# marcin119a/vae-los-angeles

Hardware: AMD Instinct MI355X
Metric: training samples/sec, MultiModalVAE batch 65536 (higher is better)
Workload: dtype bf16

## Files before the change

### include/mmvae_hip.h

```cpp
#ifndef MMVAE_HIP_H
#define MMVAE_HIP_H
#include <stdint.h>

#ifdef __cplusplus
extern "C" {
#endif

#define MMVAE_OK 0
#define MMVAE_ERR_ARG (-1)
#define MMVAE_ERR_DTYPE (-2)

enum { MMVAE_F32 = 0, MMVAE_BF16 = 1 };
enum { MMVAE_PREC_F32 = 0, MMVAE_PREC_BF16 = 1 };
enum { MMVAE_PRO_NONE = 0, MMVAE_PRO_BN_RELU_DROP = 1, MMVAE_PRO_BN_BWD_APPLY = 2 };
enum { MMVAE_EPI_STORE = 0, MMVAE_EPI_RELU_MASK = 1, MMVAE_EPI_BN_BWD = 2, MMVAE_EPI_LOSS_MSE = 3, MMVAE_EPI_LOSS_BCE_LOGIT = 4 };
enum { MMVAE_ACT_NONE = 0, MMVAE_ACT_RELU = 1, MMVAE_ACT_SIGMOID = 2 };

#define MMVAE_TILE 128

int mmvae_abi_version(void);
int mmvae_set_tuning(int32_t key, int32_t value);

typedef struct {
    const float* src; void* dst;
// ... 101 lines not shown
    const void* w; int64_t ldw; const float* bias;
} mmvae_latent_enc;
typedef struct {
    int32_t prec, B, L, n_mod;
    mmvae_latent_enc enc_a, enc_b;
    const float* table; const int64_t* site; int32_t S;
    const float* eps;
    float* mu; float* logvar;
    void* z; int64_t ldz;
    const void* w_stem; int64_t ldw_stem; const float* bias_stem; int32_t N_stem;
    void* h0; int64_t ldh0;
} mmvae_latent_fwd_args;
int mmvae_latent_fwd(const mmvae_latent_fwd_args* args, void* stream);

typedef struct {
    int32_t B, A, D, S, L;
    const float* recon_a; const void* a; int64_t ld_ra, ld_a;
    const float* recon_b; const void* b; int64_t ld_rb, ld_b;
    const float* logits; int64_t ld_logits; const int64_t* site; const float* class_weights;
    const float* mu; const float* logvar;
    float beta, gamma;
    double* sums;
    void* g_a; int32_t g_a_dtype; int64_t ld_ga;
    void* g_b; int32_t g_b_dtype; int64_t ld_gb; int32_t grad_b_wrt_logit;
    float* g_c; int64_t ld_gc;
    float* g_mu; float* g_lv;
    const float* beta_gamma_dev;
    int32_t a_dtype, b_dtype;
} mmvae_loss_args;
int mmvae_vae_loss(const mmvae_loss_args* args, void* stream);
// ... 33 lines not shown
```

### vae-los-angeles_amd/csrc/common.h

```cpp
#pragma once
#include <hip/hip_runtime.h>
#include <stdint.h>
#include "mmvae_hip.h"

namespace mm {

typedef __bf16 bf16;
typedef __attribute__((ext_vector_type(8))) __bf16 bf16x8;
typedef __attribute__((ext_vector_type(4))) __bf16 bf16x4;
typedef __attribute__((ext_vector_type(4))) float f32x4;
typedef __attribute__((ext_vector_type(2))) float f32x2;
typedef __attribute__((ext_vector_type(4))) short s16x4;

constexpr int WAVE = 64;
constexpr int TILE = 128;
constexpr int NTHREADS = 256;
constexpr int ROW_BYTES = 128;

template <typename CT> struct Mma;

template <> struct Mma<bf16> {
    static constexpr int EPC = 8;
    static constexpr int KSTEP = 32;
    typedef bf16x8 frag;
// ... 124 lines not shown
#define STAMP_ENTRY()
#endif


struct Tuning {
    int nt_wide_min_m = 256 * 128;
    int nt2_on = 1;
    long split_bytes = 1L << 32;
    long block_bytes = 1L << 31;
    int tn_wide_on = 1;
    int bnbwd_stream = 1;
    int relu_stream = 1;
    int ntp_on = 1;
    int ntp_min_m = 16384;
    int latent_on = 1;
};
inline Tuning g_tuning;

constexpr int NOT_TAKEN = 1 << 30;

template <auto Kernel, typename... Args>
inline int launch_lds(dim3 grid, dim3 block, int lds, hipStream_t st, const Args&... args) {
    static bool attr_done = false;
    if (!attr_done) {
        hipError_t e = hipFuncSetAttribute((const void*)Kernel, hipFuncAttributeMaxDynamicSharedMemorySize, lds);
        if (e != hipSuccess) return (int)e;
        attr_done = true;
    }
    hipLaunchKernelGGL(Kernel, grid, block, lds, st, args...);
    return (int)hipGetLastError();
// ... 49 lines not shown
```

### vae-los-angeles_amd/csrc/elementwise.hip

```cpp
#include <vector>
#include "common.h"
#include "mmvae_hip.h"
#include "fuse_math.h"

namespace mm {

__global__ __launch_bounds__(256) void prep_weights_kernel(const mmvae_prep_item* __restrict__ items) {
    const mmvae_prep_item it = items[blockIdx.y];
    __shared__ float tile[32][33];
    const int tx = threadIdx.x & 31, ty = threadIdx.x >> 5;
    const int tiles_c = (it.dst_cols + 31) / 32, tiles_r = (it.dst_rows + 31) / 32;
    auto put = [&](int r, int c, float v) {
        if (it.dst_dtype == MMVAE_BF16) ((bf16*)it.dst)[(long)r * it.dst_ld + c] = (bf16)v;
        else ((float*)it.dst)[(long)r * it.dst_ld + c] = v;
    };
    for (int t = blockIdx.x; t < tiles_r * tiles_c; t += gridDim.x) {
        const int tr = t / tiles_c, tc = t - tr * tiles_c;
        if (it.transpose) {
#pragma unroll
            for (int k = 0; k < 4; ++k) {
                const int sr = tc * 32 + ty + 8 * k, sc = tr * 32 + tx;
                tile[ty + 8 * k][tx] = (sr < it.src_rows && sc < it.src_cols) ? it.src[(long)sr * it.src_ld + sc] : 0.f;
            }
            __syncthreads();
// ... 226 lines not shown
            const long i = min(i0 + (long)u * blockDim.x, iend - 1);
            const int b = (int)(i / a.L), l = (int)(i - (long)b * a.L);
            bb[u] = b; ll[u] = l;
            dz[u] = a.dz[(long)b * a.lddz + l];
            if (a.dz2) dz[u] += a.dz2[(long)b * a.lddz + l];
            if (a.dz3) dz[u] += a.dz3[(long)b * a.lddz + l];
            gm[u] = a.g_mu ? a.g_mu[i] : 0.f; gl[u] = a.g_lv ? a.g_lv[i] : 0.f;
            ep[u] = a.eps[i]; lv[u] = a.logvar[i];
            sidx[u] = a.d_table ? a.site[b] : 0;
            if (sidx[u] < 0 || sidx[u] >= a.S) sidx[u] = -1;
        }
#pragma unroll
        for (int u = 0; u < U; ++u) {
            if (i0 + (long)u * blockDim.x >= iend) break;
            const int b = bb[u], l = ll[u];
            float dmu = gm[u] + dz[u];
            float dlv = gl[u] + dz[u] * ep[u] * expf(0.5f * lv[u]) * 0.5f;
            if (a.n_mod > 1) { dmu *= inv_n; dlv *= inv_n; }
            a.d_heads[(long)b * a.ld_heads + l] = dmu;
            a.d_heads[(long)b * a.ld_heads + a.L + l] = dlv;
            if (a.d_heads_lp) {
                bf16* lp = (bf16*)a.d_heads_lp + (long)b * a.ld_heads_lp;
                lp[l] = (bf16)dmu; lp[a.L + l] = (bf16)dlv;
                if (l == 0) for (int e = 2 * a.L; e < a.ld_heads_lp; ++e) lp[e] = (bf16)0.f;
            }
            if (a.d_table && sidx[u] >= 0) {
                const long sx = sidx[u];
                if (use_lds) { atomicAdd(&sT[sx * L2 + l], dmu); atomicAdd(&sT[sx * L2 + a.L + l], dlv); }
                else { unsafeAtomicAdd(&dtab[sx * L2 + l], dmu); unsafeAtomicAdd(&dtab[sx * L2 + a.L + l], dlv); }
            }
        }
    }
    if (use_lds && a.d_table) {
// ... 736 lines not shown
```

### vae-los-angeles_amd/csrc/fuse_math.h

```cpp
#pragma once
#include "common.h"

namespace mm {

__device__ __forceinline__ float fuse_reparam_elem(float& mu, float& lv, int n_mod, float inv_n, float eps) {
    if (n_mod > 1) { mu *= inv_n; lv *= inv_n; }
    return mu + eps * expf(0.5f * lv);
}

}
```

### vae-los-angeles_amd/csrc/gemm_nt.hip

```cpp
#include "common.h"
#include "mmvae_hip.h"
#include "gemm_src.h"
#include "gemm_nt_epi.h"
#include "gemm_nt2.h"

namespace mm {

STAMP_BUFFER(nt)

__device__ __forceinline__ int swz(int row, int chunk) { return row * ROW_BYTES + ((chunk ^ (row & 7)) << 4); }

template <int WN> struct NtLds {
    static constexpr int BUF = (TILE + 64 * WN) * ROW_BYTES;
    static constexpr int STAGE = 2 * BUF;
    static constexpr int ECOL = STAGE + 4096 + 4 * 64 * WN * 4;
    static constexpr int TOTAL = ECOL + 8 * 64 * WN * 4;
};

template <typename CT, typename Src, typename Epi, int WN>
__global__ __launch_bounds__(128 * WN, 2)
void gemm_nt_kernel(Src src, const CT* __restrict__ W, long ldw, int M, int N, int K, int gx, int gy, Epi epi)
{
    constexpr int EPC = Mma<CT>::EPC;
    constexpr int BK = ROW_BYTES / (int)sizeof(CT);
// ... 292 lines not shown
    mm::Tuning& t = mm::g_tuning;
    switch (key) {
    case 0: t.nt_wide_min_m = value; return 0;
    case 2: t.nt2_on = value; return 0;
    case 3:
        if (value != 0 && (value < 17 || value > 32)) return MMVAE_ERR_ARG;
        t.split_bytes = value ? 1L << value : mm::Tuning{}.split_bytes;
        t.block_bytes = t.split_bytes / 2;
        return 0;
    case 4: t.tn_wide_on = value; return 0;
    case 6: t.bnbwd_stream = value; return 0;
    case 7: t.relu_stream = value; return 0;
    case 8: t.ntp_on = value; return 0;
    case 9: t.ntp_min_m = value; return 0;
    case 10: t.latent_on = value; return 0;
    }
    return MMVAE_ERR_ARG;
}

extern "C" int mmvae_gemm_nt(const mmvae_gemm_nt_args* a, void* stream) {
    if (!a || !a->a || !a->w || (!a->c && !(a->epilogue == MMVAE_EPI_BN_BWD && a->bn_phase == 0))) return MMVAE_ERR_ARG;
    if (a->M <= 0 || a->N <= 0 || a->K <= 0) return MMVAE_ERR_ARG;
    if (a->ldw % 64 || ((uintptr_t)a->w & 15)) return MMVAE_ERR_ARG;
    const long lim = 1L << 32;
    if (((long)a->N + 256) * a->ldw * 4 >= lim) return MMVAE_ERR_ARG;
    const long a_row = (long)a->lda * (a->a_dtype == MMVAE_BF16 ? 2 : 4);
    long row_bytes = a_row > (long)a->ld_pro_mask ? a_row : (long)a->ld_pro_mask;
    if (!mm::bn_fin_ok(a)) return MMVAE_ERR_ARG;
    if (mm::needs_row_blocks(a->M, row_bytes)) {
        if (a->pro_finalize || a->pro_out) return MMVAE_ERR_ARG;
// ... 23 lines not shown
```

### vae-los-angeles_amd/csrc/latent.hip

```cpp
#include "common.h"
#include "mmvae_hip.h"
#include "gemm_src.h"
#include "fuse_math.h"

namespace mm {

constexpr int LAT_WAVES = 8, LAT_THREADS = 64 * LAT_WAVES;
constexpr int LAT_NK = 8;
constexpr int LAT_HN = 48;
constexpr int LAT_FU = LAT_HN / 2 * 16 / 64;
constexpr int LAT_NS = 448;
constexpr int LAT_MAXTAB = 1024;
constexpr int LAT_WROW = LAT_NK * 64 + 16;
constexpr int LAT_SROW = 64 + 16;
constexpr int LAT_SUMLD = 52;
constexpr int LAT_OFF_WS = 2 * LAT_HN * LAT_WROW;
constexpr int LAT_OFF_AUX = LAT_OFF_WS + LAT_NS * LAT_SROW;
constexpr int LAT_OFF_BIAS = LAT_OFF_AUX + 2 * 4096;
constexpr int LAT_OFF_TAB = LAT_OFF_BIAS + (2 * LAT_HN + LAT_NS) * 4;
constexpr int LAT_OFF_SCR = LAT_OFF_TAB + LAT_MAXTAB * 4;
constexpr int LAT_SCR_Z = 16 * LAT_SUMLD * 4;
constexpr int LAT_SCR = LAT_SCR_Z + 16 * LAT_SROW;
constexpr int LAT_LDS = LAT_OFF_SCR + LAT_WAVES * LAT_SCR;

// ... 182 lines not shown
    o = LatEnc{};
    if (!e.y) return 0;
    const mmvae_bn_finalize_args* f = (const mmvae_bn_finalize_args*)e.finalize;
    if (e.K < 32 || e.K % 32 || e.K > 32 * LAT_NK || e.ldy % 8 || e.ldy < e.K || ((uintptr_t)e.y & 15)) return MMVAE_ERR_ARG;
    if (!e.w || e.ldw % 64 || e.ldw < e.K || ((uintptr_t)e.w & 15)) return MMVAE_ERR_ARG;
    if (!f && (!e.scale || !e.shift)) return MMVAE_ERR_ARG;
    if (f && (f->N != e.K || f->M != B || B < 2 || !f->sum || !f->sumsq || !f->gamma || !f->beta || !f->mean || !f->rstd || !f->scale || !f->shift))
        return MMVAE_ERR_ARG;
    if (e.mask && (e.ld_mask % 8 || e.ld_mask < e.K || ((uintptr_t)e.mask & 7))) return MMVAE_ERR_ARG;
    const long lim = 1L << 32;
    if ((long)B * e.ldy * 2 >= lim || (e.mask && (long)B * e.ld_mask >= lim)) return MMVAE_ERR_ARG;
    o.src = SrcBnReluDrop<bf16>{(const bf16*)e.y, e.ldy, B, e.K, e.scale, e.shift, e.mask, e.ld_mask, e.inv_keep, bn_fin_from(f)};
    o.w = (const bf16*)e.w; o.ldw = e.ldw; o.bias = e.bias; o.nk = e.K / 32;
    return 0;
}

}

extern "C" int mmvae_latent_fwd(const mmvae_latent_fwd_args* a, void* stream) {
    using namespace mm;
    if (!a || !g_tuning.latent_on) return MMVAE_ERR_ARG;
    if (a->prec != MMVAE_PREC_BF16) return MMVAE_ERR_DTYPE;
    if (a->B <= 0 || a->L <= 0 || 2 * a->L > LAT_HN || (long)a->B * a->L >= (1L << 31)) return MMVAE_ERR_ARG;
    if (!a->eps || !a->mu || !a->logvar || !a->z || !a->w_stem || !a->h0) return MMVAE_ERR_ARG;
    const int present = (a->enc_a.y != nullptr) + (a->enc_b.y != nullptr) + (a->table != nullptr);
    if (present == 0 || present != a->n_mod) return MMVAE_ERR_ARG;
    if (a->table && (!a->site || a->S <= 0 || (long)a->S * 2 * a->L > LAT_MAXTAB)) return MMVAE_ERR_ARG;
    if (a->ldz % 8 || a->ldz < a->L || a->ldz > 32 || ((uintptr_t)a->z & 15)) return MMVAE_ERR_ARG;
    if (a->N_stem < 64 || a->N_stem % 64 || a->N_stem > LAT_NS || a->ldw_stem % 64 || a->ldw_stem < 32 || ((uintptr_t)a->w_stem & 15)) return MMVAE_ERR_ARG;
    if (a->ldh0 % 64 || a->ldh0 < a->N_stem || ((uintptr_t)a->h0 & 127) || (long)a->B * a->ldh0 * 2 >= (1L << 32)) return MMVAE_ERR_ARG;
    LatArgs k{};
    { const int rc = lat_enc(a->enc_a, a->B, k.e[0]); if (rc) return rc; }
    { const int rc = lat_enc(a->enc_b, a->B, k.e[1]); if (rc) return rc; }
    k.B = a->B; k.L = a->L; k.n_mod = a->n_mod; k.S = a->S;
    k.table = a->table; k.site = (const long long*)a->site; k.eps = a->eps; k.mu = a->mu; k.logvar = a->logvar;
    k.z = (bf16*)a->z; k.ldz = a->ldz;
    k.ws = (const bf16*)a->w_stem; k.ldws = a->ldw_stem; k.bs = a->bias_stem; k.ns = a->N_stem;
    k.h0 = (bf16*)a->h0; k.ldh0 = a->ldh0;
    k.nslabs = (a->B + 15) / 16;
    int grid = (k.nslabs + LAT_WAVES - 1) / LAT_WAVES;
    if (grid > 256) grid = 256;
    return launch_lds<latent_fwd_kernel>(dim3(grid), dim3(LAT_THREADS), LAT_LDS, (hipStream_t)stream, k);
}
```

### vae-los-angeles_amd/mmvae/_lib.py

```python
import ctypes as C
import os

_HERE = os.path.dirname(os.path.abspath(__file__))
LIB_PATH = os.environ.get("MMVAE_LIB_PATH") or os.path.join(_HERE, "libmmvae_hip.so")
ABI_VERSION = 20

F32, BF16 = 0, 1
PREC_F32, PREC_BF16 = 0, 1
PRO_NONE, PRO_BN_RELU_DROP, PRO_BN_BWD_APPLY = 0, 1, 2
TABLE_COPIES = 8
EPI_STORE, EPI_RELU_MASK, EPI_BN_BWD, EPI_LOSS_MSE, EPI_LOSS_BCE_LOGIT = 0, 1, 2, 3, 4
ACT_NONE, ACT_RELU, ACT_SIGMOID = 0, 1, 2
TILE = 128
TN_GROUP_MAX = 8
CTR_COPIES = 16384

i32, i64, f32, vp = C.c_int32, C.c_int64, C.c_float, C.c_void_p


class PrepItem(C.Structure):
    _fields_ = [("src", vp), ("dst", vp), ("src_rows", i32), ("src_cols", i32), ("src_ld", i64),
                ("dst_rows", i32), ("dst_cols", i32), ("dst_ld", i64), ("transpose", i32), ("dst_dtype", i32)]


# ... 52 lines not shown

class LatentEnc(C.Structure):
    _fields_ = [("y", vp), ("ldy", i64), ("K", i32), ("scale", vp), ("shift", vp),
                ("mask", vp), ("ld_mask", i64), ("inv_keep", f32), ("finalize", vp),
                ("w", vp), ("ldw", i64), ("bias", vp)]


class LatentFwdArgs(C.Structure):
    _fields_ = [("prec", i32), ("B", i32), ("L", i32), ("n_mod", i32),
                ("enc_a", LatentEnc), ("enc_b", LatentEnc),
                ("table", vp), ("site", vp), ("S", i32),
                ("eps", vp), ("mu", vp), ("logvar", vp),
                ("z", vp), ("ldz", i64),
                ("w_stem", vp), ("ldw_stem", i64), ("bias_stem", vp), ("N_stem", i32),
                ("h0", vp), ("ldh0", i64)]


class FuseBwdArgs(C.Structure):
    _fields_ = [("B", i32), ("L", i32), ("n_mod", i32),
                ("g_mu", vp), ("g_lv", vp), ("dz", vp), ("dz2", vp), ("dz3", vp), ("lddz", i64),
                ("eps", vp), ("logvar", vp),
                ("d_heads", vp), ("ld_heads", i64),
                ("d_table", vp), ("site", vp), ("S", i32), ("d_heads_lp", vp), ("ld_heads_lp", i64), ("table_copies", i32)]


class LossArgs(C.Structure):
    _fields_ = [("B", i32), ("A", i32), ("D", i32), ("S", i32), ("L", i32),
                ("recon_a", vp), ("a", vp), ("ld_ra", i64), ("ld_a", i64),
                ("recon_b", vp), ("b", vp), ("ld_rb", i64), ("ld_b", i64),
                ("logits", vp), ("ld_logits", i64), ("site", vp), ("class_weights", vp),
# ... 18 lines not shown
    "mmvae_set_tuning": [i32, i32],
    "mmvae_prep_weights": [vp, i32, vp],
    "mmvae_gemm_nt": [C.POINTER(GemmNtArgs), vp],
    "mmvae_gemm_tn": [C.POINTER(GemmTnArgs), vp],
    "mmvae_gemm_tn_group": [vp, i32, vp],
    "mmvae_bn_finalize": [C.POINTER(BnFinalizeArgs), vp],
    "mmvae_bn_eval_coeffs": [i32, vp, vp, vp, vp, f32, vp, vp, vp, vp, vp],
    "mmvae_bn_bwd_finalize": [C.POINTER(BnBwdFinalizeArgs), vp],
    "mmvae_bn_bwd_apply": [i32, i32, i32, vp, i64, vp, i64, vp, vp, vp, vp],
    "mmvae_bn_bwd_finalize_apply": [i32, i32, i32, vp, i64, vp, i64, vp, vp, vp, vp, vp, vp, vp, i32, vp],
    "mmvae_embed_table_fwd": [i32, i32, i32, vp, vp, vp, vp, vp, vp, vp],
    "mmvae_embed_table_bwd": [i32, i32, i32, vp, vp, vp, vp, i32, vp, vp, vp, vp, vp, vp],
    "mmvae_fuse_reparam_fwd": [C.POINTER(FuseFwdArgs), vp],
    "mmvae_fuse_reparam_bwd": [C.POINTER(FuseBwdArgs), vp],
    "mmvae_latent_fwd": [C.POINTER(LatentFwdArgs), vp],
    "mmvae_vae_loss": [C.POINTER(LossArgs), vp],
    "mmvae_loss_finalize": [vp, f32, f32, vp, vp, vp],
    "mmvae_gather_rows": [vp, i32, vp, i32, i64, vp],
    "mmvae_rows_to_bf16": [vp, i32, i64, vp, i64, i32, i32, vp],
    "mmvae_sigmoid_bwd": [i32, i32, vp, i64, vp, i64, vp, i32, i64, vp],
    "mmvae_scale_if_needed": [vp, i32, i64, vp, vp],
    "mmvae_scale_many": [C.POINTER(ScaleItem), i32, vp, vp],
    "mmvae_noise": [vp, i64, f32, vp, i64, C.c_uint64, C.c_uint64, vp, i32, vp],
    "mmvae_counter_add": [vp, C.c_uint64, vp],
    "mmvae_adamw_step": [vp, i32, f32, f32, f32, f32, f32, f32, f32, i32, vp, i32, vp, vp],
}
EXPORTED = ["mmvae_abi_version"] + sorted(_SIGNATURES)

_lib = None

# ... 37 lines not shown
```

### vae-los-angeles_amd/mmvae/engine.py

```python
import os
from dataclasses import dataclass
from typing import NamedTuple, Optional

import torch

from . import ops
from . import _lib as L_
from .ops import (PREC_BF16, PREC_F32, ACT_NONE, ACT_RELU, ACT_SIGMOID, EPI_RELU_MASK, EPI_BN_BWD, DROP_P,
                  ceil_to, act_dtype, Prologue, BnBwdEpilogue, BnBwdFinalize, BnBwdApply)

_PRECISIONS = {"bf16": PREC_BF16, "fp32": PREC_F32, "f32": PREC_F32}
_default_precision = _PRECISIONS[os.environ.get("MMVAE_PRECISION", "bf16").lower()]
_TINY_DW_MAX = 16384


def set_default_precision(name):
    global _default_precision
    _default_precision = _PRECISIONS[name.lower()]


def default_precision():
    return _default_precision


# ... 237 lines not shown
            else:
                ops.gemm_nt(prec, h, pl.w, N, K, y, bias=pl.bias, prologue=pro, tag=f"{self.name}.L{len(layers)}.fwd")
                ops.bn_eval_coeffs(bn.weight, bn.bias, bn.running_mean, bn.running_var, st.scale, st.shift, bn.eps, st.mean, st.rstd)
                new_pro = Prologue(st.scale, st.shift, None, 1.0)
            layers.append(LayerSave(h, pro, y, st, new_pro) if h_act is None else LayerSave(h_act, None, y, st, new_pro))
            h, pro = y, new_pro
        owed = ops.LatentEncoder(h, pro, fin, self.pl_heads)
        return (self.run_heads(prec, owed) if heads else owed), layers

    def run_heads(self, prec, owed):
        heads = torch.empty(owed.y.shape[0], 2 * self.latent, dtype=torch.float32, device=owed.y.device)
        self._consume(prec, owed.y, owed.prologue, owed.fin, 2 * self.latent, self.pl_heads.K, heads, self.pl_heads.bias, self.pl_heads.w,
                      f"{self.name}.heads.fwd")
        return heads

    def backward(self, prec, layers, d_heads, grads, tn=ops.gemm_tn, stats_bufs=None, train=True, d_heads_lp=None):
        B, dev = d_heads.shape[0], d_heads.device
        adt = act_dtype(prec)
        L2 = 2 * self.latent
        Kl = self.pl_heads.K
        gw = grads[self.fc_mu.weight]
        gb = grads[self.fc_mu.bias]
        tn(prec, d_heads, layers[-1].y, _span(gw, L2 * Kl).view(L2, Kl), _span(gb, L2), L2, Kl, q_prologue=layers[-1].y_prologue, tag=f"{self.name}.heads.dW")
        src, src_wt, src_n, src_k = (d_heads_lp if d_heads_lp is not None else d_heads), self.pl_heads.wt, Kl, L2
        for i in reversed(range(len(self.linears))):
            lin, bn, pl = self.linears[i], self.bns[i], self.pl[i]
            sv = layers[i]
            y = sv.y
            st = sv.bn
            N, K = pl.N, pl.K
            bnargs = BnBwdEpilogue(st.scale, st.shift, st.mean, st.rstd, sv.y_prologue.mask, sv.y_prologue.inv_keep)
            stats = stats_bufs[i] if stats_bufs is not None else torch.zeros(2, N, dtype=torch.float64, device=dev)
            coef = torch.empty(3, N, dtype=torch.float32, device=dev)
            d = torch.empty(B, ceil_to(N, 8), dtype=adt, device=dev)
            ops.gemm_nt(prec, src, src_wt, src_n, src_k, d, epilogue=EPI_BN_BWD, h=y, bn=bnargs, bn_phase=2, stats=stats, tag=f"{self.name}.L{i}.dX")
            fin = BnBwdFinalize(stats, bn.weight, grads[bn.weight], grads[bn.bias], not train)
            if i == 0 and K <= 4096:
                if prec == PREC_BF16 and B >= 8192 and N >= 128 and K >= 256:
                    try:
                        tn(prec, d, sv.q, grads[lin.weight], grads[lin.bias], N, K, q_prologue=sv.q_prologue,
                           p_prologue=BnBwdApply(y, st.mean, st.rstd, fin=fin), tag=f"{self.name}.L{i}.dW")
                        continue
                    except L_.MMVAEArgError:
                        pass
                ops.bn_bwd_finalize(B, N, stats, bn.weight, st.rstd, grads[bn.weight], grads[bn.bias], coef, eval_mode=not train)
                tn(prec, d, sv.q, grads[lin.weight], grads[lin.bias], N, K, q_prologue=sv.q_prologue,
                   p_prologue=BnBwdApply(y, st.mean, st.rstd, coef), tag=f"{self.name}.L{i}.dW")
                continue
            try:
                ops.bn_bwd_finalize_apply(d, y, B, N, st.mean, st.rstd, *fin)
# ... 288 lines not shown
        stem = self.dec_stem if all(g is not None for g in g_outs) else None
        D0, off = None, 0
        if stem is not None:
            D0 = torch.empty(B, stem.N, dtype=act_dtype(prec), device=dev)
        for dec, (acts, out), g, is_logit in zip(self.decoders, state.dec, g_outs, g_logit_flags):
            if g is None:
                continue
            if stem is not None:
                n0 = dec.linears[0].out_features
                dec.backward(prec, acts, out, g, is_logit, None, grads, tn, d0_out=D0[:, off:off + n0])
                off += n0
                continue
            dz = torch.empty(B, Ld, dtype=torch.float32, device=dev)
            dec.backward(prec, acts, out, g, is_logit, dz, grads, tn)
            dzs.append(dz)
        if stem is not None:
            dz = torch.empty(B, Ld, dtype=torch.float32, device=dev)
            ops.gemm_nt(prec, D0, stem.wt, stem.K, stem.N, dz, tag="Decoders.L0.dX")
            dzs.append(dz)
        if not dzs:
            dzs.append(torch.zeros(B, Ld, dtype=torch.float32, device=dev))
        if self.grad_sync is not None:
            self.grad_sync.early(flat, self.early_cut())
        d_heads = torch.empty(B, 2 * Ld, dtype=torch.float32, device=dev)
        d_heads_lp = torch.empty(B, ceil_to(2 * Ld, 8), dtype=torch.bfloat16, device=dev) if prec == PREC_BF16 else None
        ops.fuse_reparam_bwd(B, Ld, state.n_mod, g_mu, g_lv, dzs, state.eps, state.logvar, d_heads, zeros.d_table, site, d_heads_lp=d_heads_lp)
        if state.enc_a is not None:
            self.enc_a.backward(prec, state.enc_a, d_heads, grads, tn, zeros.bwd_stats[:n_a], train=state.train, d_heads_lp=d_heads_lp)
        if state.enc_b is not None:
            self.enc_b.backward(prec, state.enc_b, d_heads, grads, tn, zeros.bwd_stats[n_a:], train=state.train, d_heads_lp=d_heads_lp)
        if site is not None:
            self.enc_c.backward(zeros.d_table, grads)
        flush_tiny("tiny_dW.heads")
        if self.grad_sync is not None:
            self.grad_sync.final(flat)
        return flat, grads
```

### vae-los-angeles_amd/mmvae/ops.py

```python
import ctypes as C
from collections import namedtuple

import torch

from . import _lib as L
from ._lib import (F32, BF16, PREC_F32, PREC_BF16, PRO_NONE, PRO_BN_RELU_DROP, PRO_BN_BWD_APPLY, EPI_STORE, EPI_RELU_MASK,
                   EPI_BN_BWD, EPI_LOSS_MSE, EPI_LOSS_BCE_LOGIT, ACT_NONE, ACT_RELU, ACT_SIGMOID, TILE)

DROP_P = 0.1
BN_EPS, BN_MOMENTUM = 1e-5, 0.1


class KernelProbe:

    def __init__(self, only=None):
        self.records = {}
        self.only = only

    def wants(self, tag):
        return tag is not None and (self.only is None or tag in self.only)

    def begin(self):
        ev = torch.cuda.Event(enable_timing=True)
        ev.record(torch.cuda.current_stream())
# ... 403 lines not shown
    a.z, a.ldz = z.data_ptr(), _ld(z)
    a.w_stem, a.ldw_stem, a.bias_stem, a.N_stem = stem.w.data_ptr(), stem.w.stride(0), _p(stem.bias), stem.N
    a.h0, a.ldh0 = h0.data_ptr(), _ld(h0)
    return a, B * nbytes


def latent_fwd(prec, B, Ld, enc_a, enc_b, table, site, eps, mu, logvar, z, stem, h0):
    for t in (eps, mu, logvar):
        if tuple(t.shape) != (B, Ld) or not t.is_contiguous():
            raise ValueError(f"latent_fwd: eps / mu / logvar must be contiguous ({B}, {Ld}), got {tuple(t.shape)} / {t.stride()}")
    a, nbytes = latent_fwd_args(prec, B, Ld, enc_a, enc_b, table, site, eps, mu, logvar, z, stem, h0)
    with stream_span("latent.fwd", nbytes):
        L.check(L.load().mmvae_latent_fwd(C.byref(a), _stream()), "mmvae_latent_fwd")


def fuse_reparam_bwd(B, Ld, n_mod, g_mu, g_lv, dzs, eps, logvar, d_heads, d_table, site, d_heads_lp=None):
    dzs = list(dzs) + [None] * (3 - len(dzs))
    copies = d_table.shape[0] if (d_table is not None and d_table.dim() == 3) else 1
    a = L.FuseBwdArgs(B, Ld, n_mod, _p(g_mu), _p(g_lv), dzs[0].data_ptr(), _p(dzs[1]), _p(dzs[2]), _ld(dzs[0]), eps.data_ptr(), logvar.data_ptr(),
                      d_heads.data_ptr(), _ld(d_heads), _p(d_table), _p(site), d_table.shape[-2] if d_table is not None else 0,
                      _p(d_heads_lp), _ld(d_heads_lp) if d_heads_lp is not None else 0, copies)
    n_dz = sum(1 for d in dzs if d is not None)
    with stream_span("fuse_reparam_bwd", B * Ld * 4 * (n_dz + (g_mu is not None) + (g_lv is not None) + 2 + 2)):
        L.check(L.load().mmvae_fuse_reparam_bwd(C.byref(a), _stream()), "mmvae_fuse_reparam_bwd")


def loss_workspace(device):
    buf = torch.zeros(5 * 8 + 5 * 4 + 4, dtype=torch.uint8, device=device)
    return buf[:40].view(torch.float64), buf[40:60].view(torch.float32)

# ... 122 lines not shown
```

Measured before the change: 53.08 million.

## Fuse latent backward: stem dX, reparam bwd, and encoder last-layer BN-bwd dX

Adds a persistent latent_bwd kernel that computes the decoder-stem dX (dz) with MFMA, applies the reparameterisation backward, writes d_heads and site-table gradients, and immediately multiplies by the encoder head weights with the BN-backward epilogue. This produces the last encoder layer's dX and BN statistics in a single pass, without materialising dz, d_heads_lp or separate GEMM launches. It aims to cut memory traffic and launch count for small latent dims at large batch, at the cost of a large LDS footprint and a complex kernel, with fallback to the old path on argument errors.

```diff
diff --git a/include/mmvae_hip.h b/include/mmvae_hip.h
--- a/include/mmvae_hip.h
+++ b/include/mmvae_hip.h
@@ -139,6 +139,25 @@
 int mmvae_latent_fwd(const mmvae_latent_fwd_args* args, void* stream);
 
 typedef struct {
+    const void* y; int64_t ldy; int32_t K;
+    const uint8_t* mask; int64_t ld_mask; float inv_keep;
+    const float* scale; const float* shift; const float* mean; const float* rstd;
+    const void* wt; int64_t ldwt;
+    void* d; int64_t ldd;
+    double* sum_d; double* sum_dx;
+} mmvae_latent_bwd_enc;
+typedef struct {
+    int32_t prec, B, L, n_mod;
+    const void* d0; int64_t ldd0; int32_t N_stem;
+    const void* wt_stem; int64_t ldwt_stem;
+    const float* g_mu; const float* g_lv; const float* eps; const float* logvar;
+    mmvae_latent_bwd_enc enc_a, enc_b;
+    float* d_heads;
+    float* d_table; const int64_t* site; int32_t S; int32_t table_copies;
+} mmvae_latent_bwd_args;
+int mmvae_latent_bwd(const mmvae_latent_bwd_args* args, void* stream);
+
+typedef struct {
     int32_t B, A, D, S, L;
     const float* recon_a; const void* a; int64_t ld_ra, ld_a;
     const float* recon_b; const void* b; int64_t ld_rb, ld_b;
diff --git a/vae-los-angeles_amd/csrc/common.h b/vae-los-angeles_amd/csrc/common.h
--- a/vae-los-angeles_amd/csrc/common.h
+++ b/vae-los-angeles_amd/csrc/common.h
@@ -162,6 +162,7 @@
     int ntp_on = 1;
     int ntp_min_m = 16384;
     int latent_on = 1;
+    int latent_bwd_on = 1;
 };
 inline Tuning g_tuning;
 
diff --git a/vae-los-angeles_amd/csrc/elementwise.hip b/vae-los-angeles_amd/csrc/elementwise.hip
--- a/vae-los-angeles_amd/csrc/elementwise.hip
+++ b/vae-los-angeles_amd/csrc/elementwise.hip
@@ -264,9 +264,8 @@
         for (int u = 0; u < U; ++u) {
             if (i0 + (long)u * blockDim.x >= iend) break;
             const int b = bb[u], l = ll[u];
-            float dmu = gm[u] + dz[u];
-            float dlv = gl[u] + dz[u] * ep[u] * expf(0.5f * lv[u]) * 0.5f;
-            if (a.n_mod > 1) { dmu *= inv_n; dlv *= inv_n; }
+            float dmu, dlv;
+            fuse_reparam_bwd_elem(gm[u], gl[u], dz[u], ep[u], lv[u], a.n_mod, inv_n, dmu, dlv);
             a.d_heads[(long)b * a.ld_heads + l] = dmu;
             a.d_heads[(long)b * a.ld_heads + a.L + l] = dlv;
             if (a.d_heads_lp) {
diff --git a/vae-los-angeles_amd/csrc/fuse_math.h b/vae-los-angeles_amd/csrc/fuse_math.h
--- a/vae-los-angeles_amd/csrc/fuse_math.h
+++ b/vae-los-angeles_amd/csrc/fuse_math.h
@@ -8,4 +8,11 @@
     return mu + eps * expf(0.5f * lv);
 }
 
+__device__ __forceinline__ void fuse_reparam_bwd_elem(float gm, float gl, float dz, float eps, float lv, int n_mod, float inv_n,
+                                                      float& dmu, float& dlv) {
+    dmu = gm + dz;
+    dlv = gl + dz * eps * expf(0.5f * lv) * 0.5f;
+    if (n_mod > 1) { dmu *= inv_n; dlv *= inv_n; }
 }
+
+}
diff --git a/vae-los-angeles_amd/csrc/gemm_nt.hip b/vae-los-angeles_amd/csrc/gemm_nt.hip
--- a/vae-los-angeles_amd/csrc/gemm_nt.hip
+++ b/vae-los-angeles_amd/csrc/gemm_nt.hip
@@ -330,6 +330,7 @@
     case 8: t.ntp_on = value; return 0;
     case 9: t.ntp_min_m = value; return 0;
     case 10: t.latent_on = value; return 0;
+    case 12: t.latent_bwd_on = value; return 0;
     }
     return MMVAE_ERR_ARG;
 }
diff --git a/vae-los-angeles_amd/csrc/latent.hip b/vae-los-angeles_amd/csrc/latent.hip
--- a/vae-los-angeles_amd/csrc/latent.hip
+++ b/vae-los-angeles_amd/csrc/latent.hip
@@ -1,6 +1,7 @@
 #include "common.h"
 #include "mmvae_hip.h"
 #include "gemm_src.h"
+#include "gemm_nt_epi.h"
 #include "fuse_math.h"
 
 namespace mm {
@@ -220,6 +221,335 @@
     o.w = (const bf16*)e.w; o.ldw = e.ldw; o.bias = e.bias; o.nk = e.K / 32;
     return 0;
 }
+
+constexpr int LB_NJ = LAT_NS / 32;
+constexpr int LB_NP = LAT_NK / 2;
+constexpr int LB_KMAX = 64 * LB_NP;
+constexpr int LB_SROW = LAT_NS * 2 + 16;
+constexpr int LB_HROW = 128 + 16;
+constexpr int LB_DZLD = 36;
+constexpr int LB_OFF_WH = 32 * LB_SROW;
+constexpr int LB_OFF_COL = LB_OFF_WH + 2 * LB_KMAX * LB_HROW;
+constexpr int LB_OFF_STAT = LB_OFF_COL + 2 * 4 * LB_KMAX * 4;
+constexpr int LB_OFF_TAB = LB_OFF_STAT + 2 * 2 * LB_KMAX * 8;
+constexpr int LB_OFF_SCR = LB_OFF_TAB + LAT_MAXTAB * 4;
+constexpr int LB_SCR_DH = 16 * LB_DZLD * 4;
+constexpr int LB_SCR = LB_SCR_DH + 16 * LB_HROW;
+constexpr int LB_LDS = LB_OFF_SCR + LAT_WAVES * LB_SCR;
+static_assert(LB_LDS <= 160 * 1024 && LB_OFF_STAT % 8 == 0 && LB_OFF_SCR % 16 == 0, "LDS plan of latent_bwd_kernel");
+
+struct LatBEnc {
+    const bf16* y; long ldy; const uint8_t* mask; long ldm; float inv_keep;
+    const float* scale; const float* shift; const float* mean; const float* rstd;
+    const bf16* wt; long ldwt; bf16* d; long ldd; double* s1; double* s2;
+    int K;
+    int lines;
+};
+struct LatBArgs {
+    LatBEnc e[2];
+    int B, L, n_mod, S, copies, ns, nslabs;
+    const bf16* d0; long ldd0; const bf16* ws; long ldws;
+    const float* g_mu; const float* g_lv; const float* eps; const float* logvar;
+    float* d_heads; float* d_table; const long long* site;
+};
+
+__device__ __forceinline__ int lat_here(int v) { asm volatile("" : "+v"(v)); return v; }
+
+template <int CTRL> __device__ __forceinline__ float lat_dpp(float v) {
+    return __builtin_bit_cast(float, __builtin_amdgcn_mov_dpp(__builtin_bit_cast(int, v), CTRL, 0xf, 0xf, true));
+}
+template <int HALF, int CTRL> __device__ __forceinline__ void lat_rs_step(float (&v)[16], unsigned up) {
+#pragma unroll
+    for (int i = 0; i < HALF; ++i) {
+        const unsigned lo = __float_as_uint(v[i]), hi = __float_as_uint(v[i + HALF]);
+        const float keep = __uint_as_float((hi & up) | (lo & ~up));
+        const float send = __uint_as_float((lo & up) | (hi & ~up));
+        v[i] = keep + lat_dpp<CTRL>(send);
+    }
+}
+
+template <int NPA, int NPB>
+__global__ __launch_bounds__(LAT_THREADS) void latent_bwd_kernel(const LatBArgs a) {
+    constexpr int NPE[2] = {NPA, NPB};
+    extern __shared__ __attribute__((aligned(16))) unsigned char smem[];
+    const int tid = threadIdx.x, lane = tid & 63, wid = __builtin_amdgcn_readfirstlane(tid >> 6);
+    const int li_ = lane & 15, lg_ = lane >> 4;
+    int li = li_, lg = lg_;
+    float* const scol = (float*)(smem + LB_OFF_COL);
+    double* const sstat = (double*)(smem + LB_OFF_STAT);
+    float* const stab = (float*)(smem + LB_OFF_TAB);
+    unsigned char* const scr = smem + LB_OFF_SCR + wid * LB_SCR;
+    float* const sdz = (float*)scr;
+    unsigned char* const sdh = scr + LB_SCR_DH;
+    const int L = a.L, L2 = 2 * a.L;
+    const int nj = a.ns >> 5;
+    const bool two = L > 16;
+
+    int fr[LAT_FU], fl[LAT_FU];
+#pragma unroll
+    for (int i = 0; i < LAT_FU; ++i) { const int x = lane + 64 * i; fr[i] = x / L; fl[i] = x - fr[i] * L; }
+    const float inv_n = 1.f / (float)a.n_mod;
+    const int total = a.B * L;
+
+    uint4 d0r[LB_NJ];
+    uint4 yr[2][LB_NP][2];
+    uint2 mr[2][LB_NP][2];
+    float eps_r[LAT_FU], lv_r[LAT_FU], gm_r[LAT_FU], gl_r[LAT_FU];
+    long long site_r = 0;
+#pragma unroll
+    for (int i = 0; i < LAT_FU; ++i) { gm_r[i] = 0.f; gl_r[i] = 0.f; }
+    auto fetch_d0 = [&](int slab) __attribute__((always_inline)) {
+        const bf16* p = a.d0 + (long)min(slab * 16 + li, a.B - 1) * a.ldd0 + 8 * lg;
+#pragma unroll
+        for (int j = 0; j < LB_NJ; ++j)
+            if (j < nj) d0r[j] = *(const uint4*)(p + 32 * j);
+    };
+    auto fetch_el = [&](int slab) __attribute__((always_inline)) {
+#pragma unroll
+        for (int i = 0; i < LAT_FU; ++i) {
+            const int idx = min(slab * 16 * L + lane + 64 * i, total - 1);
+            eps_r[i] = a.eps[idx]; lv_r[i] = a.logvar[idx];
+        }
+        if (a.g_mu) {
+#pragma unroll
+            for (int i = 0; i < LAT_FU; ++i) gm_r[i] = a.g_mu[min(slab * 16 * L + lane + 64 * i, total - 1)];
+        }
+        if (a.g_lv) {
+#pragma unroll
+            for (int i = 0; i < LAT_FU; ++i) gl_r[i] = a.g_lv[min(slab * 16 * L + lane + 64 * i, total - 1)];
+        }
+        if (a.d_table) site_r = a.site[min(slab * 16 + (lane & 15), a.B - 1)];
+    };
+    auto fetch_y = [&](int e, int slab) __attribute__((always_inline)) {
+        const LatBEnc& E = a.e[e];
+        const long row = min(slab * 16 + li, a.B - 1);
+        const bf16* yp = E.y + row * E.ldy + 8 * lg;
+#pragma unroll
+        for (int p = 0; p < LB_NP; ++p)
+#pragma unroll
+            for (int h = 0; h < 2; ++h)
+                if (p < NPE[e] && 64 * p + 32 * h < E.K) yr[e][p][h] = *(const uint4*)(yp + 64 * p + 32 * h);
+        if (E.mask) {
+            const uint8_t* mp = E.mask + row * E.ldm + 8 * lg;
+#pragma unroll
+            for (int p = 0; p < LB_NP; ++p)
+#pragma unroll
+                for (int h = 0; h < 2; ++h)
+                    if (p < NPE[e] && 64 * p + 32 * h < E.K) mr[e][p][h] = *(const uint2*)(mp + 64 * p + 32 * h);
+        }
+    };
+
+    const int nw = gridDim.x * LAT_WAVES;
+    int slab = blockIdx.x * LAT_WAVES + wid;
+    if (slab < a.nslabs) {
+        fetch_d0(slab); fetch_el(slab);
+#pragma unroll
+        for (int e = 0; e < 2; ++e) if (NPE[e]) fetch_y(e, slab);
+    }
+
+    for (int c = tid; c < 32 * (a.ns >> 3); c += LAT_THREADS) {
+        const int r = c / (a.ns >> 3), ch = c - r * (a.ns >> 3);
+        *(uint4*)(smem + r * LB_SROW + ch * 16) = *(const uint4*)(a.ws + (long)r * a.ldws + ch * 8);
+    }
+#pragma unroll
+    for (int e = 0; e < 2; ++e) {
+        const LatBEnc& E = a.e[e];
+        if (NPE[e] == 0) continue;
+        for (int c = tid; c < NPE[e] * 64 * 8; c += LAT_THREADS) {
+            const int x = c >> 3, ch = c & 7, q = (x >> 4) & 3, i = x & 15;
+            const int wr = (x & ~63) + 32 * (q >> 1) + 8 * (i >> 2) + 4 * (q & 1) + (i & 3);
+            uint4 v = uint4{0u, 0u, 0u, 0u};
+            if (wr < E.K) v = *(const uint4*)(E.wt + (long)wr * E.ldwt + ch * 8);
+            *(uint4*)(smem + LB_OFF_WH + (e * LB_KMAX + x) * LB_HROW + ch * 16) = v;
+        }
+        for (int c = tid; c < LB_KMAX; c += LAT_THREADS) {
+            const bool ok = c < E.K;
+            float* t = scol + e * 4 * LB_KMAX + c;
+            t[0] = ok ? E.scale[c] : 0.f; t[LB_KMAX] = ok ? E.shift[c] : 0.f; t[2 * LB_KMAX] = ok ? E.mean[c] : 0.f; t[3 * LB_KMAX] = ok ? E.rstd[c] : 0.f;
+        }
+    }
+    for (int c = tid; c < 2 * 2 * LB_KMAX; c += LAT_THREADS) sstat[c] = 0.0;
+    if (a.d_table) for (int i = tid; i < a.S * L2; i += LAT_THREADS) stab[i] = 0.f;
+    for (int i = lane; i < 16 * LB_HROW / 16; i += 64) ((uint4*)sdh)[i] = uint4{0u, 0u, 0u, 0u};
+    __syncthreads();
+
+    EpiBnBwd<bf16, bf16> epi{};
+    epi.phase = 2;
+    for (; slab < a.nslabs; slab += nw) {
+        li = lat_here(li_); lg = lat_here(lg_);
+        {
+            f32x4 acc[2] = {f32x4{0.f, 0.f, 0.f, 0.f}, f32x4{0.f, 0.f, 0.f, 0.f}};
+#pragma unroll
+            for (int j = 0; j < LB_NJ; ++j) {
+                if (j >= nj) continue;
+                const bf16x8 df = __builtin_bit_cast(bf16x8, d0r[j]);
+                Mma<bf16>::mma(acc[0], *(const bf16x8*)(smem + li * LB_SROW + (4 * j + lg) * 16), df);
+                if (two) Mma<bf16>::mma(acc[1], *(const bf16x8*)(smem + (16 + li) * LB_SROW + (4 * j + lg) * 16), df);
+            }
+            *(f32x4*)(sdz + li * LB_DZLD + 4 * lg) = acc[0];
+            *(f32x4*)(sdz + li * LB_DZLD + 16 + 4 * lg) = acc[1];
+            if (a.d_table && lane < 16) ((int*)sdz)[lane * LB_DZLD + 32] = (site_r >= 0 && site_r < a.S) ? (int)site_r : -1;
+        }
+        lat_wave_sync();
+
+#pragma unroll
+        for (int i = 0; i < LAT_FU; ++i) {
+            if (lane + 64 * i >= 16 * L) break;
+            const int r = fr[i], l = fl[i];
+            const bool rok = slab * 16 * L + lane + 64 * i < total;
+            float dmu, dlv;
+            fuse_reparam_bwd_elem(gm_r[i], gl_r[i], sdz[r * LB_DZLD + l], eps_r[i], lv_r[i], a.n_mod, inv_n, dmu, dlv);
+            if (!rok) { dmu = 0.f; dlv = 0.f; }
+            else {
+                float* dh = a.d_heads + (long)(slab * 16 + r) * L2 + l;
+                dh[0] = dmu; dh[L] = dlv;
+                if (a.d_table) {
+                    const int sx = ((const int*)sdz)[r * LB_DZLD + 32];
+                    if (sx >= 0) { atomicAdd(&stab[sx * L2 + l], dmu); atomicAdd(&stab[sx * L2 + L + l], dlv); }
+                }
+            }
+            bf16* ip = (bf16*)sdh + r * (LB_HROW / 2) + l;
+            ip[0] = (bf16)dmu; ip[L] = (bf16)dlv;
+        }
+        lat_wave_sync();
+
+        const bf16x8 dh0 = *(const bf16x8*)(sdh + li * LB_HROW + lg * 16), dh1 = *(const bf16x8*)(sdh + li * LB_HROW + (4 + lg) * 16);
+        const bool rok = slab * 16 + li < a.B;
+        const int rbase = slab * 16 + (li & 7);
+        const bool ok0 = rbase < a.B, ok1 = rbase + 8 < a.B;
+#pragma unroll
+        for (int e = 0; e < 2; ++e) {
+            const LatBEnc& E = a.e[e];
+            if (NPE[e] == 0) continue;
+            epi.mask = E.mask; epi.inv_keep = E.inv_keep;
+            const float* ct = scol + e * 4 * LB_KMAX;
+            double* st = sstat + e * 2 * LB_KMAX;
+#pragma unroll
+            for (int p = 0; p < LB_NP; ++p) {
+                if (p >= NPE[e]) continue;
+                const int li = lat_here(li_), lg = lat_here(lg_);
+                const bool lowl = li < 8;
+                f32x4 acc[4];
+#pragma unroll
+                for (int q = 0; q < 4; ++q) {
+                    const unsigned char* wp = smem + LB_OFF_WH + (e * LB_KMAX + 64 * p + 16 * q + li) * LB_HROW + lg * 16;
+                    acc[q] = f32x4{0.f, 0.f, 0.f, 0.f};
+                    Mma<bf16>::mma(acc[q], *(const bf16x8*)wp, dh0);
+                    Mma<bf16>::mma(acc[q], *(const bf16x8*)(wp + 64), dh1);
+                }
+                uint32_t pk[2][4] = {};
+#pragma unroll
+                for (int h = 0; h < 2; ++h) {
+                    if (64 * p + 32 * h >= E.K) continue;
+                    const int cb = 64 * p + 32 * h + 8 * lg;
+                    const uint32_t yw[4] = {yr[e][p][h].x, yr[e][p][h].y, yr[e][p][h].z, yr[e][p][h].w};
+                    const uint32_t mw[2] = {mr[e][p][h].x, mr[e][p][h].y};
+                    float v[16], o[8];
+#pragma unroll
+                    for (int v4 = 0; v4 < 2; ++v4) {
+                        const f32x4 sc = *(const f32x4*)(ct + cb + 4 * v4), sh = *(const f32x4*)(ct + LB_KMAX + cb + 4 * v4);
+                        const f32x4 mu = *(const f32x4*)(ct + 2 * LB_KMAX + cb + 4 * v4), rs = *(const f32x4*)(ct + 3 * LB_KMAX + cb + 4 * v4);
+#pragma unroll
+                        for (int x4 = 0; x4 < 4; ++x4) {
+                            const int x = 4 * v4 + x4;
+                            const float av = acc[2 * h + v4][x4];
+                            const float yv = __uint_as_float((x & 1) ? (yw[x >> 1] & 0xffff0000u) : (yw[x >> 1] << 16));
+                            const unsigned mb = E.mask ? ((mw[v4] >> (8 * x4)) & 0xffu) : 1u;
+                            const EpiBnBwd<bf16, bf16>::Col cc{sc[x4], sh[x4], mu[x4], rs[x4], 0.f, 0.f, 0.f};
+                            float s1 = 0.f, s2 = 0.f;
+                            o[x] = epi.compute<0>(av, yv, mb, cc, rok, s1, s2);
+                            v[x] = s1; v[8 + x] = s2;
+                        }
+                    }
+#pragma unroll
+                    for (int qd = 0; qd < 4; ++qd) {
+                        typedef __attribute__((ext_vector_type(2))) __bf16 bf16x2;
+                        const bf16x2 t = {(bf16)o[2 * qd], (bf16)o[2 * qd + 1]};
+                        pk[h][qd] = __builtin_bit_cast(uint32_t, t);
+                    }
+                    if (!E.lines && rok) *(uint4*)(E.d + (long)(slab * 16 + li) * E.ldd + cb) = uint4{pk[h][0], pk[h][1], pk[h][2], pk[h][3]};
+                    lat_rs_step<8, 0x128>(v, (li & 8) ? 0xffffffffu : 0u);
+                    lat_rs_step<4, 0x141>(v, (li & 4) ? 0xffffffffu : 0u);
+                    lat_rs_step<2, 0x4e>(v, (li & 2) ? 0xffffffffu : 0u);
+                    lat_rs_step<1, 0xb1>(v, (li & 1) ? 0xffffffffu : 0u);
+                    atomicAdd(st + (li >> 3) * LB_KMAX + 64 * p + 32 * h + 8 * lg + (li & 7), (double)v[0]);
+                }
+                if (E.lines) {
+                    uint32_t st0[4], st1[4];
+#pragma unroll
+                    for (int qd = 0; qd < 4; ++qd) {
+                        const uint32_t send = lowl ? pk[1][qd] : pk[0][qd];
+                        const uint32_t got = (uint32_t)__builtin_amdgcn_mov_dpp((int)send, 0x128, 0xf, 0xf, true);
+                        st0[qd] = lowl ? pk[0][qd] : got;
+                        st1[qd] = lowl ? got : pk[1][qd];
+                    }
+                    bf16* crow = E.d + (long)rbase * E.ldd + 64 * p + 32 * (li >> 3) + 8 * lg;
+                    if (ok0) *(uint4*)crow = uint4{st0[0], st0[1], st0[2], st0[3]};
+                    if (ok1) *(uint4*)(crow + 8 * E.ldd) = uint4{st1[0], st1[1], st1[2], st1[3]};
+                }
+            }
+            if (e == 0 && slab + nw < a.nslabs) fetch_d0(slab + nw);
+        }
+        if (slab + nw < a.nslabs) {
+            if (NPA == 0) fetch_d0(slab + nw);
+            fetch_el(slab + nw);
+#pragma unroll
+            for (int e = 0; e < 2; ++e) if (NPE[e]) fetch_y(e, slab + nw);
+        }
+        lat_wave_sync();
+    }
+
+    __syncthreads();
+#pragma unroll
+    for (int e = 0; e < 2; ++e) {
+        const LatBEnc& E = a.e[e];
+        if (NPE[e] == 0) continue;
+        for (int c = tid; c < 2 * E.K; c += LAT_THREADS) {
+            const int which = c >= E.K, col = c - which * E.K;
+            unsafeAtomicAdd((which ? E.s2 : E.s1) + col, sstat[(e * 2 + which) * LB_KMAX + col]);
+        }
+    }
+    if (a.d_table) {
+        float* dtab = a.d_table + (long)(blockIdx.x % a.copies) * a.S * L2;
+        for (int i = tid; i < a.S * L2; i += LAT_THREADS) if (stab[i] != 0.f) unsafeAtomicAdd(&dtab[i], stab[i]);
+    }
+}
+
+static int latb_enc(const mmvae_latent_bwd_enc& e, int B, LatBEnc& o) {
+    o = LatBEnc{};
+    if (!e.y) return 0;
+    if (e.K < 32 || e.K % 32 || e.K > LB_KMAX || e.ldy % 8 || e.ldy < e.K || ((uintptr_t)e.y & 15)) return MMVAE_ERR_ARG;
+    if (e.mask && (e.ld_mask % 8 || e.ld_mask < e.K || ((uintptr_t)e.mask & 7))) return MMVAE_ERR_ARG;
+    if (!e.scale || !e.shift || !e.mean || !e.rstd || !e.sum_d || !e.sum_dx) return MMVAE_ERR_ARG;
+    if (!e.wt || e.ldwt % 8 || e.ldwt < 64 || ((uintptr_t)e.wt & 15)) return MMVAE_ERR_ARG;
+    if (!e.d || e.ldd % 8 || e.ldd < e.K || ((uintptr_t)e.d & 15)) return MMVAE_ERR_ARG;
+    const long lim = 1L << 32;
+    if ((long)B * e.ldy * 2 >= lim || (long)B * e.ldd * 2 >= lim || (e.mask && (long)B * e.ld_mask >= lim)) return MMVAE_ERR_ARG;
+    o.y = (const bf16*)e.y; o.ldy = e.ldy; o.mask = e.mask; o.ldm = e.ld_mask; o.inv_keep = e.inv_keep;
+    o.scale = e.scale; o.shift = e.shift; o.mean = e.mean; o.rstd = e.rstd;
+    o.wt = (const bf16*)e.wt; o.ldwt = e.ldwt; o.d = (bf16*)e.d; o.ldd = e.ldd; o.s1 = e.sum_d; o.s2 = e.sum_dx;
+    o.K = e.K;
+    o.lines = e.K % 64 == 0 && e.ldd % 64 == 0 && ((uintptr_t)e.d & 127) == 0;
+    return 0;
+}
+
+template <int NPA, int NPB>
+static int latb_launch(int grid, hipStream_t st, const LatBArgs& k) {
+    if constexpr (NPA + NPB == 0) return MMVAE_ERR_ARG;
+    else return launch_lds<latent_bwd_kernel<NPA, NPB>>(dim3(grid), dim3(LAT_THREADS), LB_LDS, st, k);
+}
+template <int NPA>
+static int latb_launch_b(int npb, int grid, hipStream_t st, const LatBArgs& k) {
+    switch (npb) {
+    case 0: return latb_launch<NPA, 0>(grid, st, k);
+    case 1: return latb_launch<NPA, 1>(grid, st, k);
+    case 2: return latb_launch<NPA, 2>(grid, st, k);
+    case 3: return latb_launch<NPA, 3>(grid, st, k);
+    case 4: return latb_launch<NPA, 4>(grid, st, k);
+    }
+    return MMVAE_ERR_ARG;
+}
+static_assert(LB_NP == 4, "latb_launch_b / mmvae_latent_bwd dispatch on 0 .. 4 blocks per encoder");
 
 }
 
@@ -248,3 +578,35 @@
     if (grid > 256) grid = 256;
     return launch_lds<latent_fwd_kernel>(dim3(grid), dim3(LAT_THREADS), LAT_LDS, (hipStream_t)stream, k);
 }
+
+extern "C" int mmvae_latent_bwd(const mmvae_latent_bwd_args* a, void* stream) {
+    using namespace mm;
+    if (!a || !g_tuning.latent_bwd_on) return MMVAE_ERR_ARG;
+    if (a->prec != MMVAE_PREC_BF16) return MMVAE_ERR_DTYPE;
+    if (a->B <= 0 || a->L <= 0 || 2 * a->L > LAT_HN || (long)a->B * 2 * a->L >= (1L << 31) || a->n_mod < 1) return MMVAE_ERR_ARG;
+    if (!a->d0 || !a->wt_stem || !a->eps || !a->logvar || !a->d_heads) return MMVAE_ERR_ARG;
+    if (a->N_stem < 64 || a->N_stem % 64 || a->N_stem > LAT_NS) return MMVAE_ERR_ARG;
+    if (a->ldd0 % 8 || a->ldd0 < a->N_stem || ((uintptr_t)a->d0 & 15) || (long)a->B * a->ldd0 * 2 >= (1L << 32)) return MMVAE_ERR_ARG;
+    if (a->ldwt_stem % 8 || a->ldwt_stem < a->N_stem || ((uintptr_t)a->wt_stem & 15)) return MMVAE_ERR_ARG;
+    if (a->d_table && (!a->site || a->S <= 0 || (long)a->S * 2 * a->L > LAT_MAXTAB || a->table_copies < 0)) return MMVAE_ERR_ARG;
+    if (!a->enc_a.y && !a->enc_b.y) return MMVAE_ERR_ARG;
+    LatBArgs k{};
+    { const int rc = latb_enc(a->enc_a, a->B, k.e[0]); if (rc) return rc; }
+    { const int rc = latb_enc(a->enc_b, a->B, k.e[1]); if (rc) return rc; }
+    k.B = a->B; k.L = a->L; k.n_mod = a->n_mod; k.S = a->S; k.copies = a->table_copies > 0 ? a->table_copies : 1;
+    k.ns = a->N_stem; k.nslabs = (a->B + 15) / 16;
+    k.d0 = (const bf16*)a->d0; k.ldd0 = a->ldd0; k.ws = (const bf16*)a->wt_stem; k.ldws = a->ldwt_stem;
+    k.g_mu = a->g_mu; k.g_lv = a->g_lv; k.eps = a->eps; k.logvar = a->logvar;
+    k.d_heads = a->d_heads; k.d_table = a->d_table; k.site = (const long long*)a->site;
+    int grid = (k.nslabs + LAT_WAVES - 1) / LAT_WAVES;
+    if (grid > 256) grid = 256;
+    const int npa = (k.e[0].K + 63) / 64, npb = (k.e[1].K + 63) / 64;
+    switch (npa) {
+    case 0: return latb_launch_b<0>(npb, grid, (hipStream_t)stream, k);
+    case 1: return latb_launch_b<1>(npb, grid, (hipStream_t)stream, k);
+    case 2: return latb_launch_b<2>(npb, grid, (hipStream_t)stream, k);
+    case 3: return latb_launch_b<3>(npb, grid, (hipStream_t)stream, k);
+    case 4: return latb_launch_b<4>(npb, grid, (hipStream_t)stream, k);
+    }
+    return MMVAE_ERR_ARG;
+}
diff --git a/vae-los-angeles_amd/mmvae/_lib.py b/vae-los-angeles_amd/mmvae/_lib.py
--- a/vae-los-angeles_amd/mmvae/_lib.py
+++ b/vae-los-angeles_amd/mmvae/_lib.py
@@ -90,6 +90,22 @@
                 ("z", vp), ("ldz", i64),
                 ("w_stem", vp), ("ldw_stem", i64), ("bias_stem", vp), ("N_stem", i32),
                 ("h0", vp), ("ldh0", i64)]
+
+
+class LatentBwdEnc(C.Structure):
+    _fields_ = [("y", vp), ("ldy", i64), ("K", i32), ("mask", vp), ("ld_mask", i64), ("inv_keep", f32),
+                ("scale", vp), ("shift", vp), ("mean", vp), ("rstd", vp),
+                ("wt", vp), ("ldwt", i64), ("d", vp), ("ldd", i64), ("sum_d", vp), ("sum_dx", vp)]
+
+
+class LatentBwdArgs(C.Structure):
+    _fields_ = [("prec", i32), ("B", i32), ("L", i32), ("n_mod", i32),
+                ("d0", vp), ("ldd0", i64), ("N_stem", i32),
+                ("wt_stem", vp), ("ldwt_stem", i64),
+                ("g_mu", vp), ("g_lv", vp), ("eps", vp), ("logvar", vp),
+                ("enc_a", LatentBwdEnc), ("enc_b", LatentBwdEnc),
+                ("d_heads", vp),
+                ("d_table", vp), ("site", vp), ("S", i32), ("table_copies", i32)]
 
 
 class FuseBwdArgs(C.Structure):
@@ -138,6 +154,7 @@
     "mmvae_fuse_reparam_fwd": [C.POINTER(FuseFwdArgs), vp],
     "mmvae_fuse_reparam_bwd": [C.POINTER(FuseBwdArgs), vp],
     "mmvae_latent_fwd": [C.POINTER(LatentFwdArgs), vp],
+    "mmvae_latent_bwd": [C.POINTER(LatentBwdArgs), vp],
     "mmvae_vae_loss": [C.POINTER(LossArgs), vp],
     "mmvae_loss_finalize": [vp, f32, f32, vp, vp, vp],
     "mmvae_gather_rows": [vp, i32, vp, i32, i64, vp],
diff --git a/vae-los-angeles_amd/mmvae/engine.py b/vae-los-angeles_amd/mmvae/engine.py
--- a/vae-los-angeles_amd/mmvae/engine.py
+++ b/vae-los-angeles_amd/mmvae/engine.py
@@ -275,7 +275,14 @@
                       f"{self.name}.heads.fwd")
         return heads
 
-    def backward(self, prec, layers, d_heads, grads, tn=ops.gemm_tn, stats_bufs=None, train=True, d_heads_lp=None):
+    def latent_bwd_operand(self, layers, stats_bufs):
+        sv = layers[-1]
+        y, st = sv.y, sv.bn
+        d = torch.empty(y.shape[0], ceil_to(self.pl[-1].N, 8), dtype=y.dtype, device=y.device)
+        bn = BnBwdEpilogue(st.scale, st.shift, st.mean, st.rstd, sv.y_prologue.mask, sv.y_prologue.inv_keep)
+        return ops.LatentBwdEncoder(y, bn, self.pl_heads, d, stats_bufs[len(layers) - 1])
+
+    def backward(self, prec, layers, d_heads, grads, tn=ops.gemm_tn, stats_bufs=None, train=True, d_heads_lp=None, d_last=None):
         B, dev = d_heads.shape[0], d_heads.device
         adt = act_dtype(prec)
         L2 = 2 * self.latent
@@ -293,8 +300,11 @@
             bnargs = BnBwdEpilogue(st.scale, st.shift, st.mean, st.rstd, sv.y_prologue.mask, sv.y_prologue.inv_keep)
             stats = stats_bufs[i] if stats_bufs is not None else torch.zeros(2, N, dtype=torch.float64, device=dev)
             coef = torch.empty(3, N, dtype=torch.float32, device=dev)
-            d = torch.empty(B, ceil_to(N, 8), dtype=adt, device=dev)
-            ops.gemm_nt(prec, src, src_wt, src_n, src_k, d, epilogue=EPI_BN_BWD, h=y, bn=bnargs, bn_phase=2, stats=stats, tag=f"{self.name}.L{i}.dX")
+            if d_last is not None and i == len(self.linears) - 1:
+                d = d_last
+            else:
+                d = torch.empty(B, ceil_to(N, 8), dtype=adt, device=dev)
+                ops.gemm_nt(prec, src, src_wt, src_n, src_k, d, epilogue=EPI_BN_BWD, h=y, bn=bnargs, bn_phase=2, stats=stats, tag=f"{self.name}.L{i}.dX")
             fin = BnBwdFinalize(stats, bn.weight, grads[bn.weight], grads[bn.bias], not train)
             if i == 0 and K <= 4096:
                 if prec == PREC_BF16 and B >= 8192 and N >= 128 and K >= 256:
@@ -613,21 +623,36 @@
             dz = torch.empty(B, Ld, dtype=torch.float32, device=dev)
             dec.backward(prec, acts, out, g, is_logit, dz, grads, tn)
             dzs.append(dz)
-        if stem is not None:
+        fuse_latent = stem is not None and prec == PREC_BF16 and (state.enc_a is not None or state.enc_b is not None)
+
+        def stem_dx():
             dz = torch.empty(B, Ld, dtype=torch.float32, device=dev)
             ops.gemm_nt(prec, D0, stem.wt, stem.K, stem.N, dz, tag="Decoders.L0.dX")
             dzs.append(dz)
-        if not dzs:
+        if stem is not None and not fuse_latent:
+            stem_dx()
+        if not dzs and not fuse_latent:
             dzs.append(torch.zeros(B, Ld, dtype=torch.float32, device=dev))
         if self.grad_sync is not None:
             self.grad_sync.early(flat, self.early_cut())
         d_heads = torch.empty(B, 2 * Ld, dtype=torch.float32, device=dev)
-        d_heads_lp = torch.empty(B, ceil_to(2 * Ld, 8), dtype=torch.bfloat16, device=dev) if prec == PREC_BF16 else None
-        ops.fuse_reparam_bwd(B, Ld, state.n_mod, g_mu, g_lv, dzs, state.eps, state.logvar, d_heads, zeros.d_table, site, d_heads_lp=d_heads_lp)
+        d_heads_lp = d_a = d_b = None
+        if fuse_latent:
+            lat_a = self.enc_a.latent_bwd_operand(state.enc_a, zeros.bwd_stats[:n_a]) if state.enc_a is not None else None
+            lat_b = self.enc_b.latent_bwd_operand(state.enc_b, zeros.bwd_stats[n_a:]) if state.enc_b is not None else None
+            try:
+                ops.latent_bwd(prec, B, Ld, state.n_mod, D0, stem, g_mu, g_lv, state.eps, state.logvar, lat_a, lat_b, d_heads, zeros.d_table, site)
+                d_a, d_b = (lat_a.d if lat_a is not None else None), (lat_b.d if lat_b is not None else None)
+            except L_.MMVAEArgError:
+                fuse_latent = False
+                stem_dx()
+        if not fuse_latent:
+            d_heads_lp = torch.empty(B, ceil_to(2 * Ld, 8), dtype=torch.bfloat16, device=dev) if prec == PREC_BF16 else None
+            ops.fuse_reparam_bwd(B, Ld, state.n_mod, g_mu, g_lv, dzs, state.eps, state.logvar, d_heads, zeros.d_table, site, d_heads_lp=d_heads_lp)
         if state.enc_a is not None:
-            self.enc_a.backward(prec, state.enc_a, d_heads, grads, tn, zeros.bwd_stats[:n_a], train=state.train, d_heads_lp=d_heads_lp)
+            self.enc_a.backward(prec, state.enc_a, d_heads, grads, tn, zeros.bwd_stats[:n_a], train=state.train, d_heads_lp=d_heads_lp, d_last=d_a)
         if state.enc_b is not None:
-            self.enc_b.backward(prec, state.enc_b, d_heads, grads, tn, zeros.bwd_stats[n_a:], train=state.train, d_heads_lp=d_heads_lp)
+            self.enc_b.backward(prec, state.enc_b, d_heads, grads, tn, zeros.bwd_stats[n_a:], train=state.train, d_heads_lp=d_heads_lp, d_last=d_b)
         if site is not None:
             self.enc_c.backward(zeros.d_table, grads)
         flush_tiny("tiny_dW.heads")
diff --git a/vae-los-angeles_amd/mmvae/ops.py b/vae-los-angeles_amd/mmvae/ops.py
--- a/vae-los-angeles_amd/mmvae/ops.py
+++ b/vae-los-angeles_amd/mmvae/ops.py
@@ -441,6 +441,48 @@
         L.check(L.load().mmvae_latent_fwd(C.byref(a), _stream()), "mmvae_latent_fwd")
 
 
+LatentBwdEncoder = namedtuple("LatentBwdEncoder", "y bn heads d stats")
+
+
+def _latent_bwd_enc(e, enc):
+    sc, sh, mean, rstd, mask, inv_keep = enc.bn
+    e.y, e.ldy, e.K = _mat(enc.y, "y").data_ptr(), _ld(enc.y), enc.heads.K
+    e.mask, e.ld_mask, e.inv_keep = _p(mask), (_ld(mask) if mask is not None else 0), inv_keep
+    e.scale, e.shift, e.mean, e.rstd = sc.data_ptr(), sh.data_ptr(), mean.data_ptr(), rstd.data_ptr()
+    e.wt, e.ldwt = enc.heads.wt.data_ptr(), enc.heads.wt.stride(0)
+    e.d, e.ldd = _mat(enc.d, "d").data_ptr(), _ld(enc.d)
+    e.sum_d, e.sum_dx = enc.stats[0].data_ptr(), enc.stats[1].data_ptr()
+
+
+def latent_bwd_args(prec, B, Ld, n_mod, D0, stem, g_mu, g_lv, eps, logvar, enc_a, enc_b, d_heads, d_table, site):
+    a = L.LatentBwdArgs()
+    a.prec, a.B, a.L, a.n_mod = prec, B, Ld, n_mod
+    a.d0, a.ldd0, a.N_stem = _mat(D0, "D0").data_ptr(), _ld(D0), stem.N
+    a.wt_stem, a.ldwt_stem = stem.wt.data_ptr(), stem.wt.stride(0)
+    a.g_mu, a.g_lv, a.eps, a.logvar = _p(g_mu), _p(g_lv), eps.data_ptr(), logvar.data_ptr()
+    nbytes = D0.element_size() * stem.N + 4 * Ld * ((g_mu is not None) + (g_lv is not None) + 2 + 2) + 8 * (d_table is not None)
+    for e, enc in ((a.enc_a, enc_a), (a.enc_b, enc_b)):
+        if enc is not None:
+            _latent_bwd_enc(e, enc)
+            nbytes += enc.heads.K * (enc.y.element_size() + (enc.bn[4] is not None) + enc.d.element_size())
+    a.d_heads = d_heads.data_ptr()
+    if d_table is not None:
+        a.d_table, a.site, a.S = d_table.data_ptr(), _p(site), d_table.shape[-2]
+        a.table_copies = d_table.shape[0] if d_table.dim() == 3 else 1
+    return a, B * nbytes
+
+
+def latent_bwd(prec, B, Ld, n_mod, D0, stem, g_mu, g_lv, eps, logvar, enc_a, enc_b, d_heads, d_table, site):
+    for t in (g_mu, g_lv, eps, logvar):
+        if t is not None and (tuple(t.shape) != (B, Ld) or not t.is_contiguous() or t.dtype != torch.float32):
+            raise ValueError(f"latent_bwd: g_mu / g_lv / eps / logvar must be contiguous fp32 ({B}, {Ld}), got {tuple(t.shape)} / {t.stride()}")
+    if tuple(d_heads.shape) != (B, 2 * Ld) or not d_heads.is_contiguous():
+        raise ValueError(f"latent_bwd: d_heads must be contiguous ({B}, {2 * Ld})")
+    a, nbytes = latent_bwd_args(prec, B, Ld, n_mod, D0, stem, g_mu, g_lv, eps, logvar, enc_a, enc_b, d_heads, d_table, site)
+    with stream_span("latent.bwd", nbytes):
+        L.check(L.load().mmvae_latent_bwd(C.byref(a), _stream()), "mmvae_latent_bwd")
+
+
 def fuse_reparam_bwd(B, Ld, n_mod, g_mu, g_lv, dzs, eps, logvar, d_heads, d_table, site, d_heads_lp=None):
     dzs = list(dzs) + [None] * (3 - len(dzs))
     copies = d_table.shape[0] if (d_table is not None and d_table.dim() == 3) else 1
```

Result: no change. 53.28 million, median of 6 (+0.4%).
